# gunrock/graphblast

Measured on NVIDIA H100. Metric: MTEPS, higher is better.
Workload: dtype f32

## Files before the change

graphblast_b200/csrc/graphblas/backend/cuda/kernels/bfs_fused.cuh:

```cuda
#ifndef GRAPHBLAS_BACKEND_CUDA_KERNELS_BFS_FUSED_CUH_
#define GRAPHBLAS_BACKEND_CUDA_KERNELS_BFS_FUSED_CUH_

#include <cooperative_groups.h>

#include "graphblas/backend/cuda/kernels/common.cuh"

namespace graphblas {
namespace backend {

#ifndef GB_BFS_NT
#define GB_BFS_NT     512
#endif
#ifndef GB_BFS_MINB
#define GB_BFS_MINB   2
#endif
#ifndef GB_BFS_PUSH_NT
#define GB_BFS_PUSH_NT   768
#endif
#ifndef GB_BFS_PUSH_MINB
#define GB_BFS_PUSH_MINB 2
#endif
#ifndef GB_BFS_BATCH
#define GB_BFS_BATCH  4
#endif
#ifndef GB_BFS_WALK_STEP
#define GB_BFS_WALK_STEP 4
#endif
#ifndef GB_BFS_WALK_WARP
#define GB_BFS_WALK_WARP 32
#endif
#ifndef GB_BFS_WALK_INLINE
#define GB_BFS_WALK_INLINE 64
#endif
#define GB_BFS_HEAVY  2048
#define GB_BFS_HEAVY_CAP 4096
#define GB_BFS_CHUNK  1024

struct BfsFusedArgs {
  const Index* push_ptr;   const Index* push_ind;
  const Index* pull_ptr;   const Index* pull_ind;
  const Index* pull_probe;
  const unsigned int* pull_empty;
  const unsigned int* push_empty;
  int   trace;
  unsigned long long* prof_bytes;
  Index n;
  Index source;
  int   max_levels;
  float switchpoint;
  int   mode;
  float*        levels;
  unsigned char* level8;
  unsigned int* visited[2];
  unsigned int* frontier;
  unsigned int* next;
  unsigned long long* counters;
  Index*        heavy;
  Index*        walk;
  int*          walk_count;
  Index*        walk_chunks;
};

#define GB_BFS_TIMED_LEVELS 16

enum BfsCell {
  GB_BFS_CELL_FOUND = 0,
  GB_BFS_CELL_HEAVY = GB_BFS_CELL_FOUND + 3,
  GB_BFS_CELL_LEVELS = GB_BFS_CELL_HEAVY + 3,
  GB_BFS_CELL_INSPECTED,
  GB_BFS_CELL_PULL_LEVELS,
  GB_BFS_CELL_PUSHED_VERTICES,
  GB_BFS_CELL_PUSHED_EDGES,
  GB_BFS_CELL_FOUND_PUSHING,
  GB_BFS_CELL_LEVEL_CLOCK,
  GB_BFS_CELL_START_CLOCK = GB_BFS_CELL_LEVEL_CLOCK + GB_BFS_TIMED_LEVELS,
  GB_BFS_CELL_END_PASS_CLOCK,
  GB_BFS_CELL_LAST_LEVEL_CLOCK,
  GB_BFS_CELL_WALK_CLAIM = 35,
  GB_BFS_CELL_LISTED = GB_BFS_CELL_WALK_CLAIM + 3,
  GB_BFS_CELL_SCAN_CLOCK = 44,
  GB_BFS_CELL_WALKED = GB_BFS_CELL_SCAN_CLOCK + GB_BFS_TIMED_LEVELS,
  GB_BFS_CELL_LISTED_CHUNKS = GB_BFS_CELL_WALKED + GB_BFS_TIMED_LEVELS,
  GB_BFS_NCOUNTERS = 128
};
static_assert(GB_BFS_CELL_LISTED_CHUNKS + GB_BFS_TIMED_LEVELS <= GB_BFS_NCOUNTERS,
              "the per-level cells of the last timed level are past the counters");

__device__ __forceinline__ unsigned long long* bfsLevelCell(unsigned long long* cells,
                                                            int first, int level) {
  return cells + first + level % 3;
}
__device__ __forceinline__ void bfsZeroNextCell(unsigned long long* cells, int first,
                                                int level) {
  cells[first + (level + 1) % 3] = 0ull;
}

__device__ __forceinline__ unsigned long long bfsClockNs() {
  unsigned long long t;
  asm volatile("mov.u64 %0, %globaltimer;" : "=l"(t));
  return t;
}

template <typename V>
__device__ __forceinline__ bool bfsClaim(unsigned int* visited, V vtx) {
  const unsigned int bit = 1u << (vtx & 31);
  unsigned int* word = visited + (vtx >> 5);
  if (*reinterpret_cast<volatile unsigned int*>(word) & bit) return false;
  return (atomicOr(word, bit) & bit) == 0;
}

__device__ __forceinline__ void bfsSetLevel(const BfsFusedArgs& a, Index row, int lv) {
  if (lv < 255) {
    a.level8[row] = static_cast<unsigned char>(lv);
  } else {
    a.level8[row] = 255;
    a.levels[row] = static_cast<float>(lv);
  }
}

__device__ __forceinline__ Index bfsClaimChunk(unsigned long long* cell, int lane) {
  unsigned long long c = 0ull;
  if (lane == 0) c = atomicAdd(cell, 1ull);
  return static_cast<Index>(__shfl_sync(GB_FULL_MASK, c, 0));
}

__device__ __forceinline__ unsigned int* bfsVis(const BfsFusedArgs& a, int vsel) {
  return vsel ? a.visited[1] : a.visited[0];
}
__device__ __forceinline__ unsigned int* bfsVisOther(const BfsFusedArgs& a, int vsel) {
  return vsel ? a.visited[0] : a.visited[1];
}
__device__ __forceinline__ unsigned int* bfsF(const BfsFusedArgs& a, int fsel) {
  return fsel ? a.next : a.frontier;
}
__device__ __forceinline__ unsigned int* bfsN(const BfsFusedArgs& a, int fsel) {
  return fsel ? a.frontier : a.next;
}

__device__ __forceinline__ unsigned int bfsIsolated(const BfsFusedArgs& a, Index w) {
  return a.pull_empty[w] & (a.push_empty != NULL ? a.push_empty[w] : 0xffffffffu);
}

__device__ __forceinline__ bool bfsWalkRows(const BfsFusedArgs& a, int vsel, Index row,
                                            bool active, int lane, int& inspected) {
  Index k = 0, end = 0;
  if (active) {
    k = __ldg(a.pull_ptr + row);
    end = __ldg(a.pull_ptr + row + 1);
  }
  const Index stop = (end - k > GB_BFS_WALK_WARP + GB_BFS_WALK_STEP)
                     ? k + GB_BFS_WALK_STEP : end;
  bool found = false;
  while (k < stop && !found) {
    Index col[GB_BFS_WALK_STEP];
    unsigned int wv[GB_BFS_WALK_STEP];
#pragma unroll
    for (int u = 0; u < GB_BFS_WALK_STEP; ++u)
      col[u] = (k + u < stop) ? __ldg(a.pull_ind + k + u) : static_cast<Index>(-1);
#pragma unroll
    for (int u = 0; u < GB_BFS_WALK_STEP; ++u)
      wv[u] = (col[u] >= 0) ? bfsVis(a, vsel)[col[u] >> 5] : 0u;
#pragma unroll
    for (int u = 0; u < GB_BFS_WALK_STEP; ++u) {
      if (found || col[u] < 0) continue;
      ++inspected;
      found = (wv[u] >> (col[u] & 31)) & 1u;
    }
    k += GB_BFS_WALK_STEP;
  }
  unsigned int longs = __ballot_sync(GB_FULL_MASK, !found && k < end);
  while (longs != 0u) {
    const int src = __ffs(longs) - 1;
    longs &= longs - 1u;
    const Index lend = __shfl_sync(GB_FULL_MASK, end, src);
    bool hit = false;
    for (Index lk = __shfl_sync(GB_FULL_MASK, k, src); lk < lend && !hit; lk += 32) {
      bool v = false;
      if (lk + lane < lend) {
        const Index col = __ldg(a.pull_ind + lk + lane);
        v = (bfsVis(a, vsel)[col >> 5] >> (col & 31)) & 1u;
      }
      const unsigned int b = __ballot_sync(GB_FULL_MASK, v);
      hit = (b != 0u);
      if (lane == 0)
        inspected += hit ? __ffs(b) : (lend - lk < 32 ? lend - lk : 32);
    }
    if (lane == src) found = hit;
  }
  return found;
}

template <int NT, int MINB, bool PULL>
__global__ void __launch_bounds__(NT, MINB)
bfsFusedKernel(BfsFusedArgs a) {
  namespace cg = cooperative_groups;
  cg::grid_group grid = cg::this_grid();
  __shared__ int s_red[NT/32];
  __shared__ unsigned int s_found[PULL ? NT/32 : 1][PULL ? 32 : 1];

  const Index n = a.n;
  const Index nwords = (n + 31) >> 5;
  const int lane = threadIdx.x & 31;
  const Index gtid = blockIdx.x*NT + threadIdx.x;
  const Index gthreads = gridDim.x*NT;
  const Index gwarp = gtid >> 5;
  const Index gwarps = gthreads >> 5;
  const Index nchunks = (nwords + 31) >> 5;

  if (gtid == 0) a.counters[GB_BFS_CELL_START_CLOCK] = bfsClockNs();
  if (gtid == 0) a.level8[a.source] = 1;
  for (Index w = gtid; w < nwords; w += gthreads) {
    const unsigned int seed = (w == (a.source >> 5)) ? (1u << (a.source & 31)) : 0u;
    a.visited[0][w] = seed | bfsIsolated(a, w);
    a.visited[1][w] = 0u; a.frontier[w] = seed; a.next[w] = 0u;
  }
  if (gtid <= GB_BFS_CELL_FOUND_PUSHING) a.counters[gtid] = 0ull;
  if (gtid >= GB_BFS_CELL_WALK_CLAIM && gtid < GB_BFS_CELL_LISTED + 3) a.counters[gtid] = 0ull;
  if (gtid >= GB_BFS_CELL_WALKED && gtid < GB_BFS_CELL_WALKED + GB_BFS_TIMED_LEVELS)
    a.counters[gtid] = 0ull;
  grid.sync();
  if (gtid == 0) a.counters[GB_BFS_CELL_LEVEL_CLOCK] = bfsClockNs() << 1;

  int vsel = 0;
  int fsel = 0;
  unsigned int fcount = 1u;
  bool dense = PULL && (a.mode == 2);
  float prev_ratio = 0.f;
  int inspected = 0;
  int pushed_vertices = 0;
  unsigned int pushed_edges = 0u;
  int pull_levels = 0;
  int level = 1;

  for (; level <= a.max_levels && fcount > 0u; ++level) {
    if (PULL && a.mode == 0) {
      const float ratio = static_cast<float>(fcount)/static_cast<float>(n);
      if (!dense) {
        if (ratio > a.switchpoint && ratio > prev_ratio) dense = true; else prev_ratio = ratio;
      } else {
        if (ratio <= a.switchpoint && ratio < prev_ratio) dense = false; else prev_ratio = ratio;
      }
    }
    unsigned long long* const count_cell = bfsLevelCell(a.counters, GB_BFS_CELL_FOUND, level);
    unsigned long long* const heavy_cell = bfsLevelCell(a.counters, GB_BFS_CELL_HEAVY, level);
    if (gtid == 0) {
      bfsZeroNextCell(a.counters, GB_BFS_CELL_FOUND, level);
      bfsZeroNextCell(a.counters, GB_BFS_CELL_HEAVY, level);
      bfsZeroNextCell(a.counters, GB_BFS_CELL_WALK_CLAIM, level);
      bfsZeroNextCell(a.counters, GB_BFS_CELL_LISTED, level);
    }
    int found_here = 0;

    if (!dense) {
      for (Index w0 = gwarp*32; w0 < nwords; w0 += gwarps*32) {
        const Index mine = w0 + lane;
        unsigned int my_bits = (mine < nwords) ? bfsF(a, fsel)[mine] : 0u;
        if (my_bits != 0u) bfsF(a, fsel)[mine] = 0u;
        unsigned int pending = __ballot_sync(GB_FULL_MASK, my_bits != 0u);
        while (pending != 0u) {
          const int src_lane = __ffs(pending) - 1;
          pending &= pending - 1u;
          unsigned int bits = __shfl_sync(GB_FULL_MASK, my_bits, src_lane);
          const Index w = w0 + src_lane;
          while (bits != 0u) {
            const int b = __ffs(bits) - 1;
            bits &= bits - 1u;
            const Index u = w*32 + b;
            const Index beg = __ldg(a.push_ptr + u);
            const Index deg = __ldg(a.push_ptr + u + 1) - beg;
            if (lane == 0) { ++pushed_vertices; pushed_edges += deg; }
            if (deg > GB_BFS_HEAVY) {
              unsigned long long slot = 0ull;
              if (lane == 0) slot = atomicAdd(heavy_cell, 1ull);
              slot = __shfl_sync(GB_FULL_MASK, slot, 0);
              if (slot < GB_BFS_HEAVY_CAP) {
                if (lane == 0) a.heavy[slot] = u;
                continue;
              }
            }
            for (Index k = lane; k < deg; k += 32) {
              const Index nbr = __ldg(a.push_ind + beg + k);
              if (bfsClaim(bfsVis(a, vsel), nbr)) {
                bfsSetLevel(a, nbr, level + 1);
                atomicOr(bfsN(a, fsel) + (nbr >> 5), 1u << (nbr & 31));
                ++found_here;
              }
            }
          }
        }
      }
      grid.sync();
      const unsigned long long listed =
          *reinterpret_cast<volatile unsigned long long*>(heavy_cell);
      const int nheavy = (listed > GB_BFS_HEAVY_CAP) ? GB_BFS_HEAVY_CAP
                                                     : static_cast<int>(listed);
      if (nheavy > 0) {
        for (int h = 0; h < nheavy; ++h) {
          const Index u = a.heavy[h];
          const Index beg = __ldg(a.push_ptr + u);
          const Index deg = __ldg(a.push_ptr + u + 1) - beg;
          for (Index k = gtid; k < deg; k += gthreads) {
            const Index nbr = __ldg(a.push_ind + beg + k);
            if (bfsClaim(bfsVis(a, vsel), nbr)) {
              bfsSetLevel(a, nbr, level + 1);
              atomicOr(bfsN(a, fsel) + (nbr >> 5), 1u << (nbr & 31));
              ++found_here;
            }
          }
        }
      }
    } else if (PULL) {
      ++pull_levels;
      unsigned long long* const walk_cell =
          bfsLevelCell(a.counters, GB_BFS_CELL_WALK_CLAIM, level);
      unsigned long long* const list_cell = bfsLevelCell(a.counters, GB_BFS_CELL_LISTED, level);
      Index c = gwarp;
      unsigned int next_vis = (c < nchunks && c*32 + lane < nwords)
                              ? bfsVis(a, vsel)[c*32 + lane] : 0xffffffffu;
      while (c < nchunks) {
        const Index word = c*32 + lane;
        const unsigned int my_vis = next_vis;
        const Index c_next = c + gwarps;
        next_vis = (c_next < nchunks && c_next*32 + lane < nwords)
                   ? bfsVis(a, vsel)[c_next*32 + lane] : 0xffffffffu;
        Index* const walk = a.walk + c*GB_BFS_CHUNK;
        int nwalk = 0;
        unsigned int my_out = 0u;
        unsigned int open = __ballot_sync(GB_FULL_MASK, my_vis != 0xffffffffu);
        unsigned int my_open = ~my_vis;
        if (word == nwords - 1 && (n & 31) != 0) my_open &= (1u << (n & 31)) - 1u;
        const int nopen = __popc(my_open);
        int first = nopen;
#pragma unroll
        for (int off = 1; off < 32; off <<= 1) {
          const int t = __shfl_up_sync(GB_FULL_MASK, first, off);
          if (lane >= off) first += t;
        }
        const int total = __shfl_sync(GB_FULL_MASK, first, 31);
        first -= nopen;
        const int word_batches = (__popc(open) + GB_BFS_BATCH - 1)/GB_BFS_BATCH;
        const int row_batches = (total + 32*GB_BFS_BATCH - 1)/(32*GB_BFS_BATCH);
        if (2*row_batches < word_batches) {
          open = 0u;
          unsigned int* const found_bits = s_found[threadIdx.x >> 5];
          found_bits[lane] = 0u;
          __syncwarp();
          for (int r0 = 0; r0 < total; r0 += 32*GB_BFS_BATCH) {
            int local[GB_BFS_BATCH];
            Index f[GB_BFS_BATCH];
#pragma unroll
            for (int j = 0; j < GB_BFS_BATCH; ++j) {
              const int r = r0 + 32*j + lane;
              int wl = 0, base = 0;
#pragma unroll
              for (int step = 16; step > 0; step >>= 1) {
                const int fs = __shfl_sync(GB_FULL_MASK, first, wl + step);
                if (fs <= r) { wl += step; base = fs; }
              }
              unsigned int m = __shfl_sync(GB_FULL_MASK, my_open, wl);
              int k = r - base, b = 0;
#pragma unroll
              for (int width = 16; width > 0; width >>= 1) {
                const int lo = __popc(m & ((1u << width) - 1u));
                if (k >= lo) { k -= lo; b += width; m >>= width; }
              }
              local[j] = wl*32 + b;
              f[j] = (r < total) ? ldStream32(a.pull_probe + c*GB_BFS_CHUNK + local[j])
                                 : static_cast<Index>(-1);
            }
            unsigned int pword[GB_BFS_BATCH];
#pragma unroll
            for (int j = 0; j < GB_BFS_BATCH; ++j)
              pword[j] = (f[j] != static_cast<Index>(-1))
                         ? bfsVis(a, vsel)[(f[j] & 0x7fffffff) >> 5] : 0u;
#pragma unroll
            for (int j = 0; j < GB_BFS_BATCH; ++j) {
              if (r0 + 32*j >= total) break;
              const bool found = (pword[j] >> (f[j] & 31)) & 1u;
              inspected += (f[j] != static_cast<Index>(-1)) ? 1 : 0;
              const bool walk_row = f[j] >= 0 && !found;
              const Index row = c*GB_BFS_CHUNK + local[j];
              const unsigned int walkers = __ballot_sync(GB_FULL_MASK, walk_row);
              if (walk_row) walk[nwalk + __popc(walkers & ((1u << lane) - 1u))] = row;
              nwalk += __popc(walkers);
              if (found) {
                atomicOr(found_bits + (local[j] >> 5), 1u << (local[j] & 31));
                bfsSetLevel(a, row, level + 1);
                ++found_here;
              }
            }
          }
          __syncwarp();
          my_out = found_bits[lane];
        }
        while (open != 0u) {
          const unsigned int batch = open;
          Index f[GB_BFS_BATCH];
#pragma unroll
          for (int j = 0; j < GB_BFS_BATCH; ++j) {
            const int wl = __ffs(open) - 1;
            open &= open - 1u;
            f[j] = static_cast<Index>(-1);
            if (wl >= 0) {
              const unsigned int m = __shfl_sync(GB_FULL_MASK, my_vis, wl);
              const Index row = c*GB_BFS_CHUNK + wl*32 + lane;
              if (row < n && !((m >> lane) & 1u)) f[j] = ldStream32(a.pull_probe + row);
            }
          }
          unsigned int pword[GB_BFS_BATCH];
#pragma unroll
          for (int j = 0; j < GB_BFS_BATCH; ++j)
            pword[j] = (f[j] != static_cast<Index>(-1))
                       ? bfsVis(a, vsel)[(f[j] & 0x7fffffff) >> 5] : 0u;
          unsigned int hit = 0u, more = 0u;
#pragma unroll
          for (int j = 0; j < GB_BFS_BATCH; ++j) {
            const bool found = (pword[j] >> (f[j] & 31)) & 1u;
            inspected += (f[j] != static_cast<Index>(-1)) ? 1 : 0;
            hit |= static_cast<unsigned int>(found) << j;
            more |= static_cast<unsigned int>(f[j] >= 0 && !found) << j;
          }
          unsigned int rest = batch;
#pragma unroll
          for (int j = 0; j < GB_BFS_BATCH && rest != 0u; ++j) {
            const int wl = __ffs(rest) - 1;
            rest &= rest - 1u;
            const Index row = c*GB_BFS_CHUNK + wl*32 + lane;
            const bool found = (hit >> j) & 1u, walk_row = (more >> j) & 1u;
            const unsigned int walkers = __ballot_sync(GB_FULL_MASK, walk_row);
            if (walk_row) walk[nwalk + __popc(walkers & ((1u << lane) - 1u))] = row;
            nwalk += __popc(walkers);
            const unsigned int out = __ballot_sync(GB_FULL_MASK, found);
            if (found) { bfsSetLevel(a, row, level + 1); ++found_here; }
            if (lane == wl) my_out = out;
          }
        }
        if (nwalk > 0 && nwalk <= GB_BFS_WALK_INLINE) {
          unsigned int* const found_bits = s_found[threadIdx.x >> 5];
          found_bits[lane] = my_out;
          __syncwarp();
          for (int i0 = 0; i0 < nwalk; i0 += 32) {
            const bool active = i0 + lane < nwalk;
            const Index row = active ? walk[i0 + lane] : 0;
            if (bfsWalkRows(a, vsel, row, active, lane, inspected)) {
              const int local = row & (GB_BFS_CHUNK - 1);
              atomicOr(found_bits + (local >> 5), 1u << (local & 31));
              bfsSetLevel(a, row, level + 1);
              ++found_here;
            }
          }
          __syncwarp();
          my_out = found_bits[lane];
        }
        if (word < nwords) {
          bfsN(a, fsel)[word] = my_out;
          bfsVisOther(a, vsel)[word] = my_vis | my_out;
          bfsF(a, fsel)[word] = 0u;
        }
        if (lane == 0 && nwalk > 0) {
          if (nwalk > GB_BFS_WALK_INLINE) {
            a.walk_count[c] = nwalk;
            a.walk_chunks[atomicAdd(list_cell, 1ull)] = c;
          }
          if (a.trace && level < GB_BFS_TIMED_LEVELS)
            atomicAdd(a.counters + GB_BFS_CELL_WALKED + level,
                      static_cast<unsigned long long>(nwalk));
        }
        c = c_next;
      }
      grid.sync();
      const Index nlisted = static_cast<Index>(
          *reinterpret_cast<volatile unsigned long long*>(list_cell));
      if (gtid == 0 && level < GB_BFS_TIMED_LEVELS) {
        a.counters[GB_BFS_CELL_SCAN_CLOCK + level] = bfsClockNs();
        if (a.trace)
          a.counters[GB_BFS_CELL_LISTED_CHUNKS + level] = static_cast<unsigned long long>(nlisted);
      }
      for (Index i = gwarp; i < nlisted; ) {
        const Index i_next = gwarps + bfsClaimChunk(walk_cell, lane);
        const Index c = a.walk_chunks[i];
        const int nwalk = a.walk_count[c];
        for (int i0 = 0; i0 < nwalk; i0 += 32) {
          const bool active = i0 + lane < nwalk;
          const Index row = active ? a.walk[c*GB_BFS_CHUNK + i0 + lane] : 0;
          if (bfsWalkRows(a, vsel, row, active, lane, inspected)) {
            const unsigned int bit = 1u << (row & 31);
            atomicOr(bfsN(a, fsel) + (row >> 5), bit);
            atomicOr(bfsVisOther(a, vsel) + (row >> 5), bit);
            bfsSetLevel(a, row, level + 1);
            ++found_here;
          }
        }
        i = i_next;
      }
    }
    const int block_found = blockSum<NT>(found_here, s_red);
    if (threadIdx.x == 0 && block_found) {
      atomicAdd(count_cell, static_cast<unsigned long long>(block_found));
      if (!dense)
        atomicAdd(a.counters + GB_BFS_CELL_FOUND_PUSHING,
                  static_cast<unsigned long long>(block_found));
    }
    grid.sync();
    if (gtid == 0 && level < GB_BFS_TIMED_LEVELS)
      a.counters[GB_BFS_CELL_LEVEL_CLOCK + level] = (bfsClockNs() << 1) | (dense ? 1ull : 0ull);
    fcount = static_cast<unsigned int>(
        *reinterpret_cast<volatile unsigned long long*>(count_cell));
    if (dense) vsel ^= 1;
    fsel ^= 1;
  }
  if (gtid == 0) a.counters[GB_BFS_CELL_LAST_LEVEL_CLOCK] = bfsClockNs();
  const unsigned int* const cut_rows = (fcount > 0u) ? bfsF(a, fsel) : NULL;
  const bool lines = (reinterpret_cast<uintptr_t>(a.levels) & 15u) == 0u;
  const Index nblocks = (nwords + 15) >> 4;
  if (PULL) {
    auto load_block = [&](Index blk, unsigned int& reached, unsigned int (&b)[4]) {
      reached = 0u;
#pragma unroll
      for (int j = 0; j < 4; ++j) b[j] = 0u;
      if (blk >= nblocks) return;
      const Index w = blk*16 + (lane & 15);
      if (lane < 16 && w < nwords) {
        reached = bfsVis(a, vsel)[w] & ~bfsIsolated(a, w);
        if (cut_rows != NULL) reached &= ~cut_rows[w];
        if (w == (a.source >> 5)) reached |= 1u << (a.source & 31);
      }
#pragma unroll
      for (int j = 0; j < 4; ++j) {
        const Index row = blk*512 + 128*j + 4*lane;
        if (lines && row + 4 <= n) b[j] = *reinterpret_cast<const unsigned int*>(a.level8 + row);
      }
    };
    unsigned int next_reached, next_b[4];
    load_block(gwarp, next_reached, next_b);
    for (Index blk = gwarp; blk < nblocks; blk += gwarps) {
      const Index r0 = blk*512;
      const unsigned int reached = next_reached;
      unsigned int lb[4];
#pragma unroll
      for (int j = 0; j < 4; ++j) lb[j] = next_b[j];
      load_block(blk + gwarps, next_reached, next_b);
#pragma unroll
      for (int j = 0; j < 4; ++j) {
        const unsigned int bits =
            (__shfl_sync(GB_FULL_MASK, reached, 4*j + (lane >> 3)) >> (4*(lane & 7))) & 0xfu;
        const Index row = r0 + 128*j + 4*lane;
        if (row >= n) continue;
        if (lines && row + 4 <= n) {
          const unsigned int b = lb[j];
          float f[4];
          bool escape = false;
#pragma unroll
          for (int k = 0; k < 4; ++k) {
            const unsigned int byte = (b >> (8*k)) & 0xffu;
            const bool r = (bits >> k) & 1u;
            escape |= r && byte == 255u;
            f[k] = r ? static_cast<float>(byte) : 0.f;
          }
          if (!escape) {
            __stcs(reinterpret_cast<float4*>(a.levels + row), make_float4(f[0], f[1], f[2], f[3]));
            continue;
          }
        }
        for (int k = 0; k < 4 && row + k < n; ++k) {
          if (!((bits >> k) & 1u)) {
            a.levels[row + k] = 0.f;
          } else {
            const unsigned int byte = a.level8[row + k];
            if (byte != 255u) a.levels[row + k] = static_cast<float>(byte);
          }
        }
      }
    }
  } else {
    for (Index blk = gwarp; blk < nblocks; blk += gwarps) {
      const Index r0 = blk*512;
      const Index w = blk*16 + (lane & 15);
      unsigned int reached = 0u;
      if (lane < 16 && w < nwords) {
        reached = bfsVis(a, vsel)[w] & ~bfsIsolated(a, w);
        if (cut_rows != NULL) reached &= ~cut_rows[w];
        if (w == (a.source >> 5)) reached |= 1u << (a.source & 31);
      }
#pragma unroll
      for (int j = 0; j < 4; ++j) {
        const unsigned int bits =
            (__shfl_sync(GB_FULL_MASK, reached, 4*j + (lane >> 3)) >> (4*(lane & 7))) & 0xfu;
        const Index row = r0 + 128*j + 4*lane;
        if (row >= n) continue;
        if (lines && row + 4 <= n) {
          const unsigned int b = *reinterpret_cast<const unsigned int*>(a.level8 + row);
          float f[4];
          bool escape = false;
#pragma unroll
          for (int k = 0; k < 4; ++k) {
            const unsigned int byte = (b >> (8*k)) & 0xffu;
            const bool r = (bits >> k) & 1u;
            escape |= r && byte == 255u;
            f[k] = r ? static_cast<float>(byte) : 0.f;
          }
          if (!escape) {
            __stcs(reinterpret_cast<float4*>(a.levels + row), make_float4(f[0], f[1], f[2], f[3]));
            continue;
          }
        }
        for (int k = 0; k < 4 && row + k < n; ++k) {
          if (!((bits >> k) & 1u)) {
            a.levels[row + k] = 0.f;
          } else {
            const unsigned int byte = a.level8[row + k];
            if (byte != 255u) a.levels[row + k] = static_cast<float>(byte);
          }
        }
      }
    }
  }
  if (a.trace) {
    grid.sync();
    if (gtid == 0) a.counters[GB_BFS_CELL_END_PASS_CLOCK] = bfsClockNs();
  }
  const int block_insp = blockSum<NT>(inspected, s_red);
  const int block_pv = blockSum<NT>(pushed_vertices, s_red);
  if (threadIdx.x == 0) {
    if (block_insp)
      atomicAdd(a.counters + GB_BFS_CELL_INSPECTED, static_cast<unsigned long long>(block_insp));
    if (block_pv)
      atomicAdd(a.counters + GB_BFS_CELL_PUSHED_VERTICES,
                static_cast<unsigned long long>(block_pv));
  }
  if (pushed_edges)
    atomicAdd(a.counters + GB_BFS_CELL_PUSHED_EDGES,
              static_cast<unsigned long long>(pushed_edges));
  if (gtid == 0) {
    a.counters[GB_BFS_CELL_LEVELS] = static_cast<unsigned long long>(level - 1);
    a.counters[GB_BFS_CELL_PULL_LEVELS] = static_cast<unsigned long long>(pull_levels);
  }
  if (a.prof_bytes != NULL) {
    if (pushed_edges) atomicAdd(a.prof_bytes, 8ull*pushed_edges);
    if (threadIdx.x == 0) {
      unsigned long long bytes = 4ull*static_cast<unsigned long long>(block_insp) +
                                 12ull*static_cast<unsigned long long>(block_pv);
      if (blockIdx.x == 0)
        bytes += static_cast<unsigned long long>(pull_levels)*
                     (12ull*static_cast<unsigned long long>(n) + 4ull) +
                 8ull*(*reinterpret_cast<volatile unsigned long long*>(
                           a.counters + GB_BFS_CELL_FOUND_PUSHING));
      if (bytes) atomicAdd(a.prof_bytes, bytes);
    }
  }
}

}
}

#endif
```

Measured before the change: 2.425 million.

## Software-pipeline pull-phase probe loads across batches and chunks

Restructures the pull-level chunk scan so the next batch's pull_probe loads, including the first batch of the next chunk, are issued before the current batch's visited-bit probes are consumed. The row-compacted and word-batched paths now share one loop. Per-batch local indices are packed into 16-bit fields to save registers. The pull-level count moves from a register to a global counter cell. The aim is to hide the dependent load latency of the probe-then-visited chain, at the cost of more live registers and more complex control flow.

Result: faster. 2.452 million (median of 6 runs) (+1.1%).

```diff
diff --git a/graphblast_b200/csrc/graphblas/backend/cuda/kernels/bfs_fused.cuh b/graphblast_b200/csrc/graphblas/backend/cuda/kernels/bfs_fused.cuh
--- a/graphblast_b200/csrc/graphblas/backend/cuda/kernels/bfs_fused.cuh
+++ b/graphblast_b200/csrc/graphblas/backend/cuda/kernels/bfs_fused.cuh
@@ -35,6 +35,7 @@
 #define GB_BFS_HEAVY  2048
 #define GB_BFS_HEAVY_CAP 4096
 #define GB_BFS_CHUNK  1024
+#define GB_BFS_LOCW   ((GB_BFS_BATCH + 1)/2)
 
 struct BfsFusedArgs {
   const Index* push_ptr;   const Index* push_ind;
@@ -141,6 +142,13 @@
   return a.pull_empty[w] & (a.push_empty != NULL ? a.push_empty[w] : 0xffffffffu);
 }
 
+__device__ __forceinline__ int bfsBatchLocal(const unsigned int (&loc)[GB_BFS_LOCW], int j) {
+  return static_cast<int>((loc[j >> 1] >> (16*(j & 1))) & 0x3ffu);
+}
+__device__ __forceinline__ int bfsBatchRounds(const unsigned int (&loc)[GB_BFS_LOCW]) {
+  return static_cast<int>(loc[0] >> 26);
+}
+
 __device__ __forceinline__ bool bfsWalkRows(const BfsFusedArgs& a, int vsel, Index row,
                                             bool active, int lane, int& inspected) {
   Index k = 0, end = 0;
@@ -229,7 +237,6 @@
   int inspected = 0;
   int pushed_vertices = 0;
   unsigned int pushed_edges = 0u;
-  int pull_levels = 0;
   int level = 1;
 
   for (; level <= a.max_levels && fcount > 0u; ++level) {
@@ -310,130 +317,185 @@
         }
       }
     } else if (PULL) {
-      ++pull_levels;
+      if (gtid == 0) ++a.counters[GB_BFS_CELL_PULL_LEVELS];
       unsigned long long* const walk_cell =
           bfsLevelCell(a.counters, GB_BFS_CELL_WALK_CLAIM, level);
       unsigned long long* const list_cell = bfsLevelCell(a.counters, GB_BFS_CELL_LISTED, level);
+      unsigned int l_my_open = 0u;
+      unsigned int l_pos = 0u;
+      int l_first = 0;
+      bool l_rows = false;
+      auto l_total = [&]() -> int {
+        return __shfl_sync(GB_FULL_MASK, l_first + __popc(l_my_open), 31);
+      };
+      auto setup_chunk = [&](Index cc, unsigned int vis) {
+        const unsigned int open = __ballot_sync(GB_FULL_MASK, vis != 0xffffffffu);
+        l_my_open = ~vis;
+        if (cc*32 + lane == nwords - 1 && (n & 31) != 0) l_my_open &= (1u << (n & 31)) - 1u;
+        const int nopen = __popc(l_my_open);
+        int first = nopen;
+#pragma unroll
+        for (int off = 1; off < 32; off <<= 1) {
+          const int t = __shfl_up_sync(GB_FULL_MASK, first, off);
+          if (lane >= off) first += t;
+        }
+        const int total = __shfl_sync(GB_FULL_MASK, first, 31);
+        l_first = first - nopen;
+        const int word_batches = (__popc(open) + GB_BFS_BATCH - 1)/GB_BFS_BATCH;
+        const int row_batches = (total + 32*GB_BFS_BATCH - 1)/(32*GB_BFS_BATCH);
+        l_rows = 2*row_batches < word_batches;
+        l_pos = l_rows ? 0u : open;
+      };
+      auto load_batch = [&](Index cc, Index (&f)[GB_BFS_BATCH],
+                            unsigned int (&loc)[GB_BFS_LOCW]) {
+        int nr = 0;
+#pragma unroll
+        for (int i = 0; i < GB_BFS_LOCW; ++i) loc[i] = 0u;
+        if (l_rows) {
+          const int r0 = static_cast<int>(l_pos);
+          const int total = l_total();
+#pragma unroll
+          for (int j = 0; j < GB_BFS_BATCH; ++j) {
+            const int r = r0 + 32*j + lane;
+            int wl = 0, base = 0;
+#pragma unroll
+            for (int step = 16; step > 0; step >>= 1) {
+              const int fs = __shfl_sync(GB_FULL_MASK, l_first, wl + step);
+              if (fs <= r) { wl += step; base = fs; }
+            }
+            unsigned int m = __shfl_sync(GB_FULL_MASK, l_my_open, wl);
+            int k = r - base, b = 0;
+#pragma unroll
+            for (int width = 16; width > 0; width >>= 1) {
+              const int lo = __popc(m & ((1u << width) - 1u));
+              if (k >= lo) { k -= lo; b += width; m >>= width; }
+            }
+            const int local = wl*32 + b;
+            loc[j >> 1] |= static_cast<unsigned int>(local) << (16*(j & 1));
+            f[j] = (r < total) ? ldStream32(a.pull_probe + cc*GB_BFS_CHUNK + local)
+                                 : static_cast<Index>(-1);
+          }
+          nr = (total - r0 + 31) >> 5;
+          if (nr > GB_BFS_BATCH) nr = GB_BFS_BATCH;
+          l_pos = static_cast<unsigned int>(r0 + 32*GB_BFS_BATCH);
+        } else {
+#pragma unroll
+          for (int j = 0; j < GB_BFS_BATCH; ++j) {
+            const int wl = __ffs(l_pos) - 1;
+            l_pos &= l_pos - 1u;
+            f[j] = static_cast<Index>(-1);
+            if (wl >= 0) {
+              ++nr;
+              const int local = wl*32 + lane;
+              loc[j >> 1] |= static_cast<unsigned int>(local) << (16*(j & 1));
+              const unsigned int m = __shfl_sync(GB_FULL_MASK, l_my_open, wl);
+              if ((m >> lane) & 1u) f[j] = ldStream32(a.pull_probe + cc*GB_BFS_CHUNK + local);
+            }
+          }
+        }
+        loc[0] |= static_cast<unsigned int>(nr) << 26;
+      };
+      auto loaded_all = [&]() -> bool {
+        return l_rows ? static_cast<int>(l_pos) >= l_total() : l_pos == 0u;
+      };
+      auto probe_batch = [&](const Index (&f)[GB_BFS_BATCH], unsigned int (&pword)[GB_BFS_BATCH]) {
+#pragma unroll
+        for (int j = 0; j < GB_BFS_BATCH; ++j)
+          pword[j] = (f[j] != static_cast<Index>(-1))
+                     ? bfsVis(a, vsel)[(f[j] & 0x7fffffff) >> 5] : 0u;
+      };
       Index c = gwarp;
-      unsigned int next_vis = (c < nchunks && c*32 + lane < nwords)
-                              ? bfsVis(a, vsel)[c*32 + lane] : 0xffffffffu;
+      unsigned int my_vis = (c < nchunks && c*32 + lane < nwords)
+                            ? bfsVis(a, vsel)[c*32 + lane] : 0xffffffffu;
+      Index f[GB_BFS_BATCH];
+      unsigned int loc[GB_BFS_LOCW];
+      if (c < nchunks) {
+        setup_chunk(c, my_vis);
+        load_batch(c, f, loc);
+      }
       while (c < nchunks) {
         const Index word = c*32 + lane;
-        const unsigned int my_vis = next_vis;
         const Index c_next = c + gwarps;
-        next_vis = (c_next < nchunks && c_next*32 + lane < nwords)
-                   ? bfsVis(a, vsel)[c_next*32 + lane] : 0xffffffffu;
+        const unsigned int next_vis = (c_next < nchunks && c_next*32 + lane < nwords)
+                                      ? bfsVis(a, vsel)[c_next*32 + lane] : 0xffffffffu;
+        const bool rows = l_rows;
         Index* const walk = a.walk + c*GB_BFS_CHUNK;
         int nwalk = 0;
         unsigned int my_out = 0u;
-        unsigned int open = __ballot_sync(GB_FULL_MASK, my_vis != 0xffffffffu);
-        unsigned int my_open = ~my_vis;
-        if (word == nwords - 1 && (n & 31) != 0) my_open &= (1u << (n & 31)) - 1u;
-        const int nopen = __popc(my_open);
-        int first = nopen;
-#pragma unroll
-        for (int off = 1; off < 32; off <<= 1) {
-          const int t = __shfl_up_sync(GB_FULL_MASK, first, off);
-          if (lane >= off) first += t;
-        }
-        const int total = __shfl_sync(GB_FULL_MASK, first, 31);
-        first -= nopen;
-        const int word_batches = (__popc(open) + GB_BFS_BATCH - 1)/GB_BFS_BATCH;
-        const int row_batches = (total + 32*GB_BFS_BATCH - 1)/(32*GB_BFS_BATCH);
-        if (2*row_batches < word_batches) {
-          open = 0u;
-          unsigned int* const found_bits = s_found[threadIdx.x >> 5];
+        unsigned int* const found_bits = s_found[threadIdx.x >> 5];
+        if (rows) {
           found_bits[lane] = 0u;
           __syncwarp();
-          for (int r0 = 0; r0 < total; r0 += 32*GB_BFS_BATCH) {
-            int local[GB_BFS_BATCH];
-            Index f[GB_BFS_BATCH];
+        }
+        unsigned int pword[GB_BFS_BATCH];
+        probe_batch(f, pword);
+        bool last;
+        do {
+          last = loaded_all();
+          Index fn[GB_BFS_BATCH];
+          unsigned int ln[GB_BFS_LOCW];
+          if (!last) {
+            load_batch(c, fn, ln);
+          } else if (c_next < nchunks) {
+            setup_chunk(c_next, next_vis);
+            load_batch(c_next, fn, ln);
+          } else {
+#pragma unroll
+            for (int j = 0; j < GB_BFS_BATCH; ++j) fn[j] = static_cast<Index>(-1);
+#pragma unroll
+            for (int i = 0; i < GB_BFS_LOCW; ++i) ln[i] = 0u;
+          }
+          if (rows) {
 #pragma unroll
             for (int j = 0; j < GB_BFS_BATCH; ++j) {
-              const int r = r0 + 32*j + lane;
-              int wl = 0, base = 0;
-#pragma unroll
-              for (int step = 16; step > 0; step >>= 1) {
-                const int fs = __shfl_sync(GB_FULL_MASK, first, wl + step);
-                if (fs <= r) { wl += step; base = fs; }
-              }
-              unsigned int m = __shfl_sync(GB_FULL_MASK, my_open, wl);
-              int k = r - base, b = 0;
-#pragma unroll
-              for (int width = 16; width > 0; width >>= 1) {
-                const int lo = __popc(m & ((1u << width) - 1u));
-                if (k >= lo) { k -= lo; b += width; m >>= width; }
-              }
-              local[j] = wl*32 + b;
-              f[j] = (r < total) ? ldStream32(a.pull_probe + c*GB_BFS_CHUNK + local[j])
-                                 : static_cast<Index>(-1);
-            }
-            unsigned int pword[GB_BFS_BATCH];
-#pragma unroll
-            for (int j = 0; j < GB_BFS_BATCH; ++j)
-              pword[j] = (f[j] != static_cast<Index>(-1))
-                         ? bfsVis(a, vsel)[(f[j] & 0x7fffffff) >> 5] : 0u;
-#pragma unroll
-            for (int j = 0; j < GB_BFS_BATCH; ++j) {
-              if (r0 + 32*j >= total) break;
+              if (j >= bfsBatchRounds(loc)) break;
+              const int local = bfsBatchLocal(loc, j);
               const bool found = (pword[j] >> (f[j] & 31)) & 1u;
               inspected += (f[j] != static_cast<Index>(-1)) ? 1 : 0;
               const bool walk_row = f[j] >= 0 && !found;
-              const Index row = c*GB_BFS_CHUNK + local[j];
+              const Index row = c*GB_BFS_CHUNK + local;
               const unsigned int walkers = __ballot_sync(GB_FULL_MASK, walk_row);
               if (walk_row) walk[nwalk + __popc(walkers & ((1u << lane) - 1u))] = row;
               nwalk += __popc(walkers);
               if (found) {
-                atomicOr(found_bits + (local[j] >> 5), 1u << (local[j] & 31));
+                atomicOr(found_bits + (local >> 5), 1u << (local & 31));
                 bfsSetLevel(a, row, level + 1);
                 ++found_here;
               }
             }
-          }
+          } else {
+            unsigned int hit = 0u, more = 0u;
+#pragma unroll
+            for (int j = 0; j < GB_BFS_BATCH; ++j) {
+              const bool found = (pword[j] >> (f[j] & 31)) & 1u;
+              inspected += (f[j] != static_cast<Index>(-1)) ? 1 : 0;
+              hit |= static_cast<unsigned int>(found) << j;
+              more |= static_cast<unsigned int>(f[j] >= 0 && !found) << j;
+            }
+#pragma unroll
+            for (int j = 0; j < GB_BFS_BATCH; ++j) {
+              if (j >= bfsBatchRounds(loc)) break;
+              const int local = bfsBatchLocal(loc, j);
+              const int wl = local >> 5;
+              const Index row = c*GB_BFS_CHUNK + local;
+              const bool found = (hit >> j) & 1u, walk_row = (more >> j) & 1u;
+              const unsigned int walkers = __ballot_sync(GB_FULL_MASK, walk_row);
+              if (walk_row) walk[nwalk + __popc(walkers & ((1u << lane) - 1u))] = row;
+              nwalk += __popc(walkers);
+              const unsigned int out = __ballot_sync(GB_FULL_MASK, found);
+              if (found) { bfsSetLevel(a, row, level + 1); ++found_here; }
+              if (lane == wl) my_out = out;
+            }
+          }
+#pragma unroll
+          for (int j = 0; j < GB_BFS_BATCH; ++j) f[j] = fn[j];
+#pragma unroll
+          for (int i = 0; i < GB_BFS_LOCW; ++i) loc[i] = ln[i];
+          if (!last) probe_batch(f, pword);
+        } while (!last);
+        if (rows) {
           __syncwarp();
           my_out = found_bits[lane];
-        }
-        while (open != 0u) {
-          const unsigned int batch = open;
-          Index f[GB_BFS_BATCH];
-#pragma unroll
-          for (int j = 0; j < GB_BFS_BATCH; ++j) {
-            const int wl = __ffs(open) - 1;
-            open &= open - 1u;
-            f[j] = static_cast<Index>(-1);
-            if (wl >= 0) {
-              const unsigned int m = __shfl_sync(GB_FULL_MASK, my_vis, wl);
-              const Index row = c*GB_BFS_CHUNK + wl*32 + lane;
-              if (row < n && !((m >> lane) & 1u)) f[j] = ldStream32(a.pull_probe + row);
-            }
-          }
-          unsigned int pword[GB_BFS_BATCH];
-#pragma unroll
-          for (int j = 0; j < GB_BFS_BATCH; ++j)
-            pword[j] = (f[j] != static_cast<Index>(-1))
-                       ? bfsVis(a, vsel)[(f[j] & 0x7fffffff) >> 5] : 0u;
-          unsigned int hit = 0u, more = 0u;
-#pragma unroll
-          for (int j = 0; j < GB_BFS_BATCH; ++j) {
-            const bool found = (pword[j] >> (f[j] & 31)) & 1u;
-            inspected += (f[j] != static_cast<Index>(-1)) ? 1 : 0;
-            hit |= static_cast<unsigned int>(found) << j;
-            more |= static_cast<unsigned int>(f[j] >= 0 && !found) << j;
-          }
-          unsigned int rest = batch;
-#pragma unroll
-          for (int j = 0; j < GB_BFS_BATCH && rest != 0u; ++j) {
-            const int wl = __ffs(rest) - 1;
-            rest &= rest - 1u;
-            const Index row = c*GB_BFS_CHUNK + wl*32 + lane;
-            const bool found = (hit >> j) & 1u, walk_row = (more >> j) & 1u;
-            const unsigned int walkers = __ballot_sync(GB_FULL_MASK, walk_row);
-            if (walk_row) walk[nwalk + __popc(walkers & ((1u << lane) - 1u))] = row;
-            nwalk += __popc(walkers);
-            const unsigned int out = __ballot_sync(GB_FULL_MASK, found);
-            if (found) { bfsSetLevel(a, row, level + 1); ++found_here; }
-            if (lane == wl) my_out = out;
-          }
         }
         if (nwalk > 0 && nwalk <= GB_BFS_WALK_INLINE) {
           unsigned int* const found_bits = s_found[threadIdx.x >> 5];
@@ -467,6 +529,7 @@
                       static_cast<unsigned long long>(nwalk));
         }
         c = c_next;
+        my_vis = next_vis;
       }
       grid.sync();
       const Index nlisted = static_cast<Index>(
@@ -633,7 +696,7 @@
               static_cast<unsigned long long>(pushed_edges));
   if (gtid == 0) {
     a.counters[GB_BFS_CELL_LEVELS] = static_cast<unsigned long long>(level - 1);
-    a.counters[GB_BFS_CELL_PULL_LEVELS] = static_cast<unsigned long long>(pull_levels);
+    if (!PULL) a.counters[GB_BFS_CELL_PULL_LEVELS] = 0ull;
   }
   if (a.prof_bytes != NULL) {
     if (pushed_edges) atomicAdd(a.prof_bytes, 8ull*pushed_edges);
@@ -641,7 +704,7 @@
       unsigned long long bytes = 4ull*static_cast<unsigned long long>(block_insp) +
                                  12ull*static_cast<unsigned long long>(block_pv);
       if (blockIdx.x == 0)
-        bytes += static_cast<unsigned long long>(pull_levels)*
+        bytes += (PULL ? a.counters[GB_BFS_CELL_PULL_LEVELS] : 0ull)*
                      (12ull*static_cast<unsigned long long>(n) + 4ull) +
                  8ull*(*reinterpret_cast<volatile unsigned long long*>(
                            a.counters + GB_BFS_CELL_FOUND_PUSHING));
```
